# daemon-219/ReID-GAN

Measured on AMD Instinct MI355X. Metric: train-step images/sec, 256×128 ReID batch, 1/2/4/8 MI355X, higher is better.
Workload: dtype f32; 1 GPU; FD-GAN G + D_id/D_pd fwd/bwd step (FDGANModel.optimize_parameters), batch 16 pairs = 32 crops of 256x128 + 18-ch pose map per GPU, stage 2, drop 0.2; crops_per_gpu=32, global_batch_crops=32, parallelism=dp1

## Files before the change

### reid-gan_amd/csrc/conv_halo.h

```cpp
#pragma once
#include "conv_finish.h"

namespace {

struct HaloP {
    ConvP c;
    int Cred;
    int HP, Wh, slab;
    int cblocks, cb_per_split;
    FastDiv d_hp, d_slab, d_wh, d_hw, d_w;
};

template <int BM, bool DGRAD, int NH>
__global__ __launch_bounds__(NT) __attribute__((amdgpu_waves_per_eu(BM == 128 ? 2 : 3))) void conv3x3_halo_kernel(const HaloP hp) {
    using T = Tile<BM, 128, 2, 2>;
    const ConvP& p = hp.c;
    __shared__ __attribute__((aligned(16))) float As[2][BK][T::LDA];
    __shared__ __attribute__((aligned(16))) float Hs[2][NH * NT];

    const int tid = threadIdx.x, lane = tid & 63, wid = tid >> 6;
    const int wm = wid >> 1, wn = wid & 1;
    const int l32 = lane & 31, kh = lane >> 5;
    const int tile = xcd_remap(blockIdx.x, gridDim.x);
    const int mt = tile % p.m_tiles, nt = tile / p.m_tiles;
    const int m0 = mt * BM, n0 = nt * 128;
    const int split = blockIdx.y;
    const int HW = p.H * p.W, HP = hp.HP, Wh = hp.Wh;
    const rsrc_t rw = make_rsrc(p.w, p.w_bytes), rx = make_rsrc(p.x, p.x_bytes);

    const int img0 = fdiv(n0, hp.d_hw);
    const int h0 = fdiv(n0 - img0 * HW, hp.d_w);

    int pos[T::TN];
#pragma unroll
    for (int j = 0; j < T::TN; ++j) {
        const int pl = wn * T::WTN + j * 32 + l32;
        const int il = fdiv(pl, hp.d_hw);
        const int rem = pl - il * HW;
        const int hl = fdiv(rem, hp.d_w);
        pos[j] = il * hp.slab + (hl + 1) * Wh + (rem - hl * p.W) + 1;
    }

    unsigned hoff[NH];
#pragma unroll
    for (int i = 0; i < NH; ++i) {
        const int f = tid + NT * i;
        const int ch = fdiv(f, hp.d_hp);
        const int ps = f - ch * HP;
        const int il = fdiv(ps, hp.d_slab);
        const int r2 = ps - il * hp.slab;
        const int hh = fdiv(r2, hp.d_wh);
        const int ww = r2 - hh * Wh - 1;
        const int img = img0 + il, h = h0 + hh - 1;
        const bool ok = ch < BK && img < p.N && (unsigned)h < (unsigned)p.H && (unsigned)ww < (unsigned)p.W;
        hoff[i] = ok ? (unsigned)((((int64_t)img * hp.Cred + ch) * p.H + h) * p.W + ww) * 4u : OOB;
    }
    const unsigned cbstride = (unsigned)(BK * HW) * 4u;

    constexpr int NA = BM / 64;
    unsigned aoff[NA];
    int arow[NA], akq[NA];
#pragma unroll
    for (int i = 0; i < NA; ++i) {
        const int v = tid + NT * i;
        if (!DGRAD) {
            arow[i] = v >> 2;
            akq[i] = (v & 3) * 4;
            aoff[i] = (m0 + arow[i] < p.M) ? (unsigned)(((int64_t)(m0 + arow[i]) * 9 * hp.Cred + akq[i]) * 4) : OOB;
        } else {
            arow[i] = v / (BM / 4);
            akq[i] = (v - arow[i] * (BM / 4)) * 4;
            aoff[i] = (m0 + akq[i] < p.M) ? (unsigned)(((int64_t)arow[i] * 9 * p.M + m0 + akq[i]) * 4) : OOB;
        }
    }
    float4 ra[NA];
    float hv[NH];
    floatx16 acc[T::TM][T::TN];
    zero_acc<T>(acc);

    auto load_a = [&](int cb, int t) {
        const unsigned kb4 = DGRAD ? (unsigned)(((int64_t)cb * BK * 9 + (8 - t)) * p.M) * 4u
                                   : (unsigned)(t * hp.Cred + cb * BK) * 4u;
#pragma unroll
        for (int i = 0; i < NA; ++i) ra[i] = bload4(rw, aoff[i] == OOB ? OOB : aoff[i] + kb4);
    };
    auto store_a = [&](int buf) {
#pragma unroll
        for (int i = 0; i < NA; ++i) {
            if (!DGRAD) {
                As[buf][akq[i] + 0][arow[i]] = ra[i].x;
                As[buf][akq[i] + 1][arow[i]] = ra[i].y;
                As[buf][akq[i] + 2][arow[i]] = ra[i].z;
                As[buf][akq[i] + 3][arow[i]] = ra[i].w;
            } else {
                *reinterpret_cast<float4*>(&As[buf][arow[i]][akq[i]]) = ra[i];
            }
        }
    };
    auto load_h = [&](int cb) {
        const unsigned o = (unsigned)cb * cbstride;
#pragma unroll
        for (int i = 0; i < NH; ++i) hv[i] = bload(rx, hoff[i] == OOB ? OOB : hoff[i] + o);
    };
    auto store_h = [&](int buf) {
#pragma unroll
        for (int i = 0; i < NH; ++i) Hs[buf][tid + NT * i] = hv[i];
    };

    const int cb_begin = split * hp.cb_per_split;
    int cb_end = cb_begin + hp.cb_per_split;
    if (cb_end > hp.cblocks) cb_end = hp.cblocks;
    if (cb_begin < cb_end) {
        load_h(cb_begin);
        load_a(cb_begin, 0);
        store_h(0);
        store_a(0);
    }
    __syncthreads();
    int ab = 0, hb = 0;
    for (int cb = cb_begin; cb < cb_end; ++cb) {
        const bool more_cb = cb + 1 < cb_end;
        for (int t = 0; t < 9; ++t) {
            const bool last = !more_cb && t == 8;
            if (t == 0 && more_cb) load_h(cb + 1);
            if (!last) load_a(t == 8 ? cb + 1 : cb, t == 8 ? 0 : t + 1);
            const int r = (t * 11) >> 5;
            const int toff = (r - 1) * Wh + (t - 3 * r - 1);
            const float* hsb = Hs[hb];
#if RG_MATH == 3
            mma_kstep<T::TM, T::TN>([&](int i, int q) { return As[ab][8 * kh + q][wm * T::WTM + i * 32 + l32]; },
                                    [&](int j, int q) { return hsb[(8 * kh + q) * HP + pos[j] + toff]; }, acc);
#else
#pragma unroll
            for (int ks = 0; ks < BK / 2; ++ks) {
                const int k = 2 * ks + kh;
                float a[T::TM], b[T::TN];
#pragma unroll
                for (int i = 0; i < T::TM; ++i) a[i] = As[ab][k][wm * T::WTM + i * 32 + l32];
#pragma unroll
                for (int j = 0; j < T::TN; ++j) b[j] = hsb[k * HP + pos[j] + toff];
#pragma unroll
                for (int i = 0; i < T::TM; ++i)
#pragma unroll
                    for (int j = 0; j < T::TN; ++j)
                        acc[i][j] = __builtin_amdgcn_mfma_f32_32x32x2f32(a[i], b[j], acc[i][j], 0, 0, 0);
            }
#endif
            if (!last) store_a(ab ^ 1);
            if (t == 8 && more_cb) store_h(hb ^ 1);
            __syncthreads();
            ab ^= 1;
        }
        hb ^= 1;
    }
    store_tile_nchw<T>(p, acc, m0, n0, wm, wn, lane, p.Ng, HW, hp.d_hw, split, nt * 2 + wn);
}

static bool halo_geom(int H, int W, int* HP, int* Wh, int* slab) {
    if (!rg::conv::switches().halo || W < 4 || W > 64 || (W & (W - 1))) return false;
    const int R = 128 / W;
    int rows, imgs;
    if (R <= H) {
        if (H % R) return false;
        rows = R;
        imgs = 1;
    } else {
        if (R % H) return false;
        rows = H;
        imgs = R / H;
    }
    *Wh = W + 2;
    *slab = (rows + 2) * (W + 2);
    *HP = imgs * *slab;
    return *HP <= 288;
}
static bool halo_geom(int H, int W) {
    int hp, wh, slab;
    return halo_geom(H, W, &hp, &wh, &slab);
}
struct HaloPlan {
    int bm, m_tiles, n_tiles, splits, per;
};
static HaloPlan halo_plan(int M, int64_t Ng, int Cred, const rg::conv::Workspace* ws) {
    HaloPlan pl;
    pl.bm = M <= 64 ? 64 : 128;
    pl.m_tiles = rg::cdiv(M, pl.bm);
    pl.n_tiles = (int)rg::cdiv64(Ng, 128);
    const int cblocks = Cred / BK;
    const int64_t tiles = (int64_t)pl.m_tiles * pl.n_tiles;
    const int target = rg::conv::switches().halo_wg;
    int64_t want = tiles >= (3 * target) / 4 ? 1 : rg::cdiv64(target, tiles);
    if (want > cblocks / 2) want = cblocks / 2;
    if (want > 16) want = 16;
    if (want < 1) want = 1;
    while (want > 1 && want * (int64_t)M * Ng * 4 >= (1ll << 31)) --want;
    pl.per = (int)rg::cdiv64(cblocks, want);
    pl.splits = rg::cdiv(cblocks, pl.per);
    if (ws && !ws->holds(rg::conv::splitk_bytes(pl.splits, M, Ng))) {
        pl.splits = 1;
        pl.per = cblocks;
    }
    return pl;
}
template <bool DGRAD>
static int halo_launch(ConvP p, int Cred, int H, int W, const HaloPlan& pl, void* workspace, hipStream_t stream, const char* op) {
    HaloP hp;
    int HPv, Wh, slab;
    halo_geom(H, W, &HPv, &Wh, &slab);
    p.m_tiles = pl.m_tiles; p.n_tiles = pl.n_tiles;
    p.splits = pl.splits;
    p.partial = pl.splits > 1 ? static_cast<float*>(workspace) : nullptr;
    p.partial_bytes = (unsigned)rg::conv::splitk_bytes(pl.splits, p.M, p.Ng);
    p.arrive = pl.splits > 1 ? splitk_arrivals(stream, pl.m_tiles * pl.n_tiles, p.partial, p.y, p.M, p.Ng, H * W, p.ep) : nullptr;
    hp.c = p;
    hp.Cred = Cred;
    hp.HP = HPv; hp.Wh = Wh; hp.slab = slab;
    hp.cblocks = Cred / BK;
    hp.cb_per_split = pl.per;
    hp.d_hp = make_fastdiv(HPv);
    hp.d_slab = make_fastdiv(slab);
    hp.d_wh = make_fastdiv(Wh);
    hp.d_hw = make_fastdiv(H * W);
    hp.d_w = make_fastdiv(W);
    const dim3 grid(pl.m_tiles * pl.n_tiles, pl.splits, 1);
    const bool small = 16 * HPv <= 13 * NT;
    if (pl.bm == 128) {
        if (small) hipLaunchKernelGGL((conv3x3_halo_kernel<128, DGRAD, 13>), grid, dim3(NT), 0, stream, hp);
        else hipLaunchKernelGGL((conv3x3_halo_kernel<128, DGRAD, 18>), grid, dim3(NT), 0, stream, hp);
    } else {
        if (small) hipLaunchKernelGGL((conv3x3_halo_kernel<64, DGRAD, 13>), grid, dim3(NT), 0, stream, hp);
        else hipLaunchKernelGGL((conv3x3_halo_kernel<64, DGRAD, 18>), grid, dim3(NT), 0, stream, hp);
    }
    if (pl.splits > 1 && !p.arrive) {
        if (int e = rg::check_launch(op)) return e;
        launch_finish(stream, p.partial, p.y, p.M, p.Ng, H * W, make_fastdiv(H * W), pl.splits, p.ep);
    }
    return rg::check_launch(op);
}

}
```

Baseline: 955.6 images/s.

## Restructure halo 3x3 conv kernel with packed LDS layout and interleaved staging

```diff
diff --git a/reid-gan_amd/csrc/conv_halo.h b/reid-gan_amd/csrc/conv_halo.h
--- a/reid-gan_amd/csrc/conv_halo.h
+++ b/reid-gan_amd/csrc/conv_halo.h
@@ -11,12 +11,26 @@
     FastDiv d_hp, d_slab, d_wh, d_hw, d_w;
 };
 
-template <int BM, bool DGRAD, int NH>
-__global__ __launch_bounds__(NT) __attribute__((amdgpu_waves_per_eu(BM == 128 ? 2 : 3))) void conv3x3_halo_kernel(const HaloP hp) {
-    using T = Tile<BM, 128, 2, 2>;
+constexpr int HL_POS = 256;
+constexpr int HL_ZERO = 256;
+constexpr int HL_HALF = HL_POS * 16;
+constexpr int HL_PIECE = HL_ZERO + 2 * HL_HALF;
+constexpr int HL_BYTES = 3 * HL_PIECE;
+
+template <int BM, bool DGRAD>
+__global__ __launch_bounds__(BM * 4) __attribute__((amdgpu_waves_per_eu(BM == 128 ? 4 : 2))) void conv3x3_halo_kernel(const HaloP hp) {
+    constexpr int NTH = BM * 4;
+    using T = Tile<BM, 128, BM / 32, 2>;
+    using LA = PlTile<DGRAD ? PL_T : PL_R, BM>;
+    static_assert(T::TM == 1 && T::TN == 2, "wave tile 32 x 64");
+    constexpr int HOFF = (2 * LA::BYTES + 255) & ~255;
+    constexpr int NUH = 2 * HL_POS / NTH;
+    constexpr int NM = 6 * T::TM * T::TN;
+    static_assert(HL_PIECE % 256 == 0 && NUH >= 1 && NUH + 4 <= NM, "aligned pieces; the micro-steps of a tap fit behind its MFMAs");
+    __shared__ __attribute__((aligned(256))) unsigned char lds[HOFF + 2 * HL_BYTES];
+    const unsigned lds0 = (unsigned)(size_t)((lds_u8_t*)lds);
+    const unsigned ldsH = lds0 + HOFF;
     const ConvP& p = hp.c;
-    __shared__ __attribute__((aligned(16))) float As[2][BK][T::LDA];
-    __shared__ __attribute__((aligned(16))) float Hs[2][NH * NT];
 
     const int tid = threadIdx.x, lane = tid & 63, wid = tid >> 6;
     const int wm = wid >> 1, wn = wid & 1;
@@ -25,133 +39,128 @@
     const int mt = tile % p.m_tiles, nt = tile / p.m_tiles;
     const int m0 = mt * BM, n0 = nt * 128;
     const int split = blockIdx.y;
-    const int HW = p.H * p.W, HP = hp.HP, Wh = hp.Wh;
+    const int HW = p.H * p.W, W = p.W;
     const rsrc_t rw = make_rsrc(p.w, p.w_bytes), rx = make_rsrc(p.x, p.x_bytes);
 
     const int img0 = fdiv(n0, hp.d_hw);
     const int h0 = fdiv(n0 - img0 * HW, hp.d_w);
-
-    int pos[T::TN];
+    const int rows2 = fdiv(hp.slab, hp.d_wh);
+    const int imgs = fdiv(hp.HP, hp.d_slab);
+    const int slabk = (imgs > 1 && HW < 32) ? HW + 16 : rows2 * W;
+
+    unsigned bpos[T::TN];
+    bool bleft[T::TN], bright[T::TN];
 #pragma unroll
     for (int j = 0; j < T::TN; ++j) {
         const int pl = wn * T::WTN + j * 32 + l32;
         const int il = fdiv(pl, hp.d_hw);
         const int rem = pl - il * HW;
-        const int hl = fdiv(rem, hp.d_w);
-        pos[j] = il * hp.slab + (hl + 1) * Wh + (rem - hl * p.W) + 1;
-    }
-
-    unsigned hoff[NH];
-#pragma unroll
-    for (int i = 0; i < NH; ++i) {
-        const int f = tid + NT * i;
-        const int ch = fdiv(f, hp.d_hp);
-        const int ps = f - ch * HP;
-        const int il = fdiv(ps, hp.d_slab);
-        const int r2 = ps - il * hp.slab;
-        const int hh = fdiv(r2, hp.d_wh);
-        const int ww = r2 - hh * Wh - 1;
+        const int w = rem & (W - 1);
+        bpos[j] = ldsH + HL_ZERO + kh * HL_HALF + (unsigned)(il * slabk + W + rem) * 16u;
+        bleft[j] = w == 0;
+        bright[j] = w == W - 1;
+    }
+
+    PlStager<NUH, 4> sh;
+    unsigned hoff[NUH];
+    {
+        const int ps = tid & (HL_POS - 1);
+        const int il = ps / slabk;
+        const int r2 = ps - il * slabk;
+        const int hh = fdiv(r2, hp.d_w);
+        const int ww = r2 - hh * W;
         const int img = img0 + il, h = h0 + hh - 1;
-        const bool ok = ch < BK && img < p.N && (unsigned)h < (unsigned)p.H && (unsigned)ww < (unsigned)p.W;
-        hoff[i] = ok ? (unsigned)((((int64_t)img * hp.Cred + ch) * p.H + h) * p.W + ww) * 4u : OOB;
+        const bool ok = il < imgs && hh < rows2 && img < p.N && (unsigned)h < (unsigned)p.H;
+#pragma unroll
+        for (int u = 0; u < NUH; ++u) {
+            const int half = NUH == 1 ? (tid >> 8) : u;
+            hoff[u] = ok ? (unsigned)((((int64_t)img * hp.Cred + 8 * half) * p.H + h) * W + ww) * 4u : OOB;
+            sh.wr[u] = ldsH + HL_ZERO + half * HL_HALF + (unsigned)ps * 16u;
+        }
     }
     const unsigned cbstride = (unsigned)(BK * HW) * 4u;
-
-    constexpr int NA = BM / 64;
-    unsigned aoff[NA];
-    int arow[NA], akq[NA];
-#pragma unroll
-    for (int i = 0; i < NA; ++i) {
-        const int v = tid + NT * i;
-        if (!DGRAD) {
-            arow[i] = v >> 2;
-            akq[i] = (v & 3) * 4;
-            aoff[i] = (m0 + arow[i] < p.M) ? (unsigned)(((int64_t)(m0 + arow[i]) * 9 * hp.Cred + akq[i]) * 4) : OOB;
-        } else {
-            arow[i] = v / (BM / 4);
-            akq[i] = (v - arow[i] * (BM / 4)) * 4;
-            aoff[i] = (m0 + akq[i] < p.M) ? (unsigned)(((int64_t)arow[i] * 9 * p.M + m0 + akq[i]) * 4) : OOB;
-        }
-    }
-    float4 ra[NA];
-    float hv[NH];
+    const unsigned chstride = (unsigned)HW * 4u;
+
+    PlStager<1, 2> sa;
+    unsigned aoff;
+    if (!DGRAD) {
+        const int row = tid >> 2, kq = (tid & 3) * 4;
+        aoff = (m0 + row < p.M) ? (unsigned)(((int64_t)(m0 + row) * 9 * hp.Cred + kq) * 4) : OOB;
+        sa.wr[0] = lds0 + LA::off_rk(row, kq);
+    } else {
+        const int krow = tid / (BM / 4), mq = (tid - krow * (BM / 4)) * 4;
+        aoff = (m0 + mq < p.M) ? (unsigned)(((int64_t)krow * 9 * p.M + m0 + mq) * 4) : OOB;
+        sa.wr[0] = lds0 + LA::off_rk(mq, krow);
+    }
+    const unsigned fa = lds0 + LA::frag_base(lane, wm * T::WTM);
+
+    float ra[4];
+    float hv[8 * NUH];
     floatx16 acc[T::TM][T::TN];
     zero_acc<T>(acc);
 
-    auto load_a = [&](int cb, int t) {
+    auto load_a = [&](int cb, int t, bool ok) {
         const unsigned kb4 = DGRAD ? (unsigned)(((int64_t)cb * BK * 9 + (8 - t)) * p.M) * 4u
                                    : (unsigned)(t * hp.Cred + cb * BK) * 4u;
-#pragma unroll
-        for (int i = 0; i < NA; ++i) ra[i] = bload4(rw, aoff[i] == OOB ? OOB : aoff[i] + kb4);
+        pl_unpack4(ra, bload4(rw, (!ok || aoff == OOB) ? OOB : aoff + kb4));
     };
-    auto store_a = [&](int buf) {
-#pragma unroll
-        for (int i = 0; i < NA; ++i) {
-            if (!DGRAD) {
-                As[buf][akq[i] + 0][arow[i]] = ra[i].x;
-                As[buf][akq[i] + 1][arow[i]] = ra[i].y;
-                As[buf][akq[i] + 2][arow[i]] = ra[i].z;
-                As[buf][akq[i] + 3][arow[i]] = ra[i].w;
-            } else {
-                *reinterpret_cast<float4*>(&As[buf][arow[i]][akq[i]]) = ra[i];
-            }
-        }
-    };
-    auto load_h = [&](int cb) {
+    auto load_h = [&](int cb, bool ok) {
         const unsigned o = (unsigned)cb * cbstride;
 #pragma unroll
-        for (int i = 0; i < NH; ++i) hv[i] = bload(rx, hoff[i] == OOB ? OOB : hoff[i] + o);
-    };
-    auto store_h = [&](int buf) {
-#pragma unroll
-        for (int i = 0; i < NH; ++i) Hs[buf][tid + NT * i] = hv[i];
+        for (int u = 0; u < NUH; ++u)
+#pragma unroll
+            for (int e = 0; e < 8; ++e) hv[8 * u + e] = bload(rx, (!ok || hoff[u] == OOB) ? OOB : hoff[u] + o + (unsigned)e * chstride);
     };
 
     const int cb_begin = split * hp.cb_per_split;
     int cb_end = cb_begin + hp.cb_per_split;
     if (cb_end > hp.cblocks) cb_end = hp.cblocks;
+
+    if (tid < 6 * (HL_ZERO / 16))
+        *(lds_int4_t*)(size_t)(ldsH + (unsigned)(tid >> 4) * HL_PIECE + (unsigned)(tid & 15) * 16u) = int4r{0, 0, 0, 0};
     if (cb_begin < cb_end) {
-        load_h(cb_begin);
-        load_a(cb_begin, 0);
-        store_h(0);
-        store_a(0);
+        load_a(cb_begin, 0, true);
+        load_h(cb_begin, true);
+#pragma unroll
+        for (int s = 0; s < decltype(sa)::STEPS; ++s) sa.step(s, ra, 0u, LA::PIECE);
+#pragma unroll
+        for (int s = 0; s < decltype(sh)::STEPS; ++s) sh.step(s, hv, 0u, HL_PIECE);
     }
     __syncthreads();
-    int ab = 0, hb = 0;
-    for (int cb = cb_begin; cb < cb_end; ++cb) {
-        const bool more_cb = cb + 1 < cb_end;
+
+    auto block = [&](auto par_tag, int cb) {
+        constexpr int PAR = decltype(par_tag)::value;
+        const bool more = cb + 1 < cb_end;
+#pragma unroll
         for (int t = 0; t < 9; ++t) {
-            const bool last = !more_cb && t == 8;
-            if (t == 0 && more_cb) load_h(cb + 1);
-            if (!last) load_a(t == 8 ? cb + 1 : cb, t == 8 ? 0 : t + 1);
-            const int r = (t * 11) >> 5;
-            const int toff = (r - 1) * Wh + (t - 3 * r - 1);
-            const float* hsb = Hs[hb];
-#if RG_MATH == 3
-            mma_kstep<T::TM, T::TN>([&](int i, int q) { return As[ab][8 * kh + q][wm * T::WTM + i * 32 + l32]; },
-                                    [&](int j, int q) { return hsb[(8 * kh + q) * HP + pos[j] + toff]; }, acc);
-#else
-#pragma unroll
-            for (int ks = 0; ks < BK / 2; ++ks) {
-                const int k = 2 * ks + kh;
-                float a[T::TM], b[T::TN];
-#pragma unroll
-                for (int i = 0; i < T::TM; ++i) a[i] = As[ab][k][wm * T::WTM + i * 32 + l32];
-#pragma unroll
-                for (int j = 0; j < T::TN; ++j) b[j] = hsb[k * HP + pos[j] + toff];
-#pragma unroll
-                for (int i = 0; i < T::TM; ++i)
-#pragma unroll
-                    for (int j = 0; j < T::TN; ++j)
-                        acc[i][j] = __builtin_amdgcn_mfma_f32_32x32x2f32(a[i], b[j], acc[i][j], 0, 0, 0);
-            }
-#endif
-            if (!last) store_a(ab ^ 1);
-            if (t == 8 && more_cb) store_h(hb ^ 1);
+            const int FB = PAR ^ (t & 1);
+            load_a(t == 8 ? cb + 1 : cb, t == 8 ? 0 : t + 1, t < 8 || more);
+            if (t == 0) load_h(cb + 1, more);
+            const int r = t / 3, s = t - 3 * r;
+            const unsigned toff = (unsigned)(((r - 1) * W + (s - 1)) * 16);
+            mma_pl<T::TM, T::TN>(
+                [&](int i, int pc) { return LA::frag(fa + FB * LA::BYTES + pc * LA::PIECE + i * LA::BLK); },
+                [&](int j, int pc) {
+                    unsigned a = bpos[j] + toff;
+                    if (s == 0) a = bleft[j] ? ldsH + (a & 0xf0u) : a;
+                    if (s == 2) a = bright[j] ? ldsH + (a & 0xf0u) : a;
+                    return *(const lds_int4_t*)(size_t)(a + PAR * HL_BYTES + pc * HL_PIECE);
+                },
+                acc,
+                [&](int slot) {
+                    if (t >= 1) {
+#pragma unroll
+                        for (int q = 0; q < NUH; ++q)
+                            if (slot == NM - 4 - NUH + q) sh.step((t - 1) * NUH + q, hv, (PAR ^ 1) * HL_BYTES, HL_PIECE);
+                    }
+                    if (slot >= NM - 4) sa.step(slot - (NM - 4), ra, (FB ^ 1) * LA::BYTES, LA::PIECE);
+                });
             __syncthreads();
-            ab ^= 1;
         }
-        hb ^= 1;
+    };
+    for (int cb = cb_begin; cb < cb_end; cb += 2) {
+        block(IntTag<0>{}, cb);
+        if (cb + 1 < cb_end) block(IntTag<1>{}, cb + 1);
     }
     store_tile_nchw<T>(p, acc, m0, n0, wm, wn, lane, p.Ng, HW, hp.d_hw, split, nt * 2 + wn);
 }
@@ -223,14 +232,8 @@
     hp.d_hw = make_fastdiv(H * W);
     hp.d_w = make_fastdiv(W);
     const dim3 grid(pl.m_tiles * pl.n_tiles, pl.splits, 1);
-    const bool small = 16 * HPv <= 13 * NT;
-    if (pl.bm == 128) {
-        if (small) hipLaunchKernelGGL((conv3x3_halo_kernel<128, DGRAD, 13>), grid, dim3(NT), 0, stream, hp);
-        else hipLaunchKernelGGL((conv3x3_halo_kernel<128, DGRAD, 18>), grid, dim3(NT), 0, stream, hp);
-    } else {
-        if (small) hipLaunchKernelGGL((conv3x3_halo_kernel<64, DGRAD, 13>), grid, dim3(NT), 0, stream, hp);
-        else hipLaunchKernelGGL((conv3x3_halo_kernel<64, DGRAD, 18>), grid, dim3(NT), 0, stream, hp);
-    }
+    if (pl.bm == 128) hipLaunchKernelGGL((conv3x3_halo_kernel<128, DGRAD>), grid, dim3(512), 0, stream, hp);
+    else hipLaunchKernelGGL((conv3x3_halo_kernel<64, DGRAD>), grid, dim3(256), 0, stream, hp);
     if (pl.splits > 1 && !p.arrive) {
         if (int e = rg::check_launch(op)) return e;
         launch_finish(stream, p.partial, p.y, p.M, p.Ng, H * W, make_fastdiv(H * W), pl.splits, p.ep);
```

Result: no change. 956.8 images/s (median of 6 runs) (+0.1%).
